# SHI-Labs/Self-Similarity-Grouping

Hardware: AMD Instinct MI355X
Metric: images/s embed + s/iter for NxN rerank+DBSCAN, N=16k, 1/2/4/8 GPU (higher is better)
Workload: dtype f32 (embed: split-half operands hi+lo on fp16 MFMA, fp32 accumulate, 6e-8 max error vs the fp32 reference features) / exact int64 via int8 MFMA digits + f64 + f16 (distance, re-rank: half semantics, bit-exact)

## Files before the change

self-similarity-grouping_amd/csrc/conv.hip:

```cpp
#include "ssg_common.h"
#include <cstdlib>
#include <type_traits>

namespace ssg {

typedef float v16f __attribute__((ext_vector_type(16)));
typedef unsigned int v4u __attribute__((ext_vector_type(4)));
typedef _Float16 v8h __attribute__((ext_vector_type(8)));

__device__ __forceinline__ unsigned pack_h2(_Float16 a, _Float16 b) {
  return (unsigned)__builtin_bit_cast(unsigned short, a) | ((unsigned)__builtin_bit_cast(unsigned short, b) << 16);
}
__device__ __forceinline__ float unpack_lo(unsigned u) { return (float)__builtin_bit_cast(_Float16, (unsigned short)(u & 0xffffu)); }
__device__ __forceinline__ float unpack_hi(unsigned u) { return (float)__builtin_bit_cast(_Float16, (unsigned short)(u >> 16)); }
__device__ __forceinline__ void split_encode4(const float4 v, uint2& hi, uint2& lo) {
  const _Float16 h0 = (_Float16)v.x, h1 = (_Float16)v.y, h2 = (_Float16)v.z, h3 = (_Float16)v.w;
  hi = make_uint2(pack_h2(h0, h1), pack_h2(h2, h3));
  lo = make_uint2(pack_h2((_Float16)(v.x - (float)h0), (_Float16)(v.y - (float)h1)), pack_h2((_Float16)(v.z - (float)h2), (_Float16)(v.w - (float)h3)));
}
__device__ __forceinline__ bool split_hi_nonfinite(const uint2 hi) {
  const unsigned a = hi.x & 0x7fff7fffu, b = hi.y & 0x7fff7fffu;
  return (a & 0xffffu) >= 0x7c00u || (a >> 16) >= 0x7c00u || (b & 0xffffu) >= 0x7c00u || (b >> 16) >= 0x7c00u;
}
__device__ __forceinline__ float4 split_decode4(const uint2 hi, const uint2 lo) {
// ... 345 lines not shown
          v.x += r4.x; v.y += r4.y; v.z += r4.z; v.w += r4.w;
        }
        if (p.relu) { v.x = v.x > 0.f ? v.x : 0.f; v.y = v.y > 0.f ? v.y : 0.f; v.z = v.z > 0.f ? v.z : 0.f; v.w = v.w > 0.f ? v.w : 0.f; }
        if (p.out_split) {
          uint2 hp, lp;
          split_encode4(v, hp, lp);
          if (p.overflow && split_hi_nonfinite(hp)) *p.overflow = 1;
          const uint2 send = odd ? hp : lp;
          const uint2 recv = make_uint2(lane_xor1(send.x), lane_xor1(send.y));
          const uint4 st = odd ? make_uint4(recv.x, recv.y, lp.x, lp.y) : make_uint4(hp.x, hp.y, recv.x, recv.y);
#ifdef SSG_IGEMM_NT_STORE
          if (m < p.M) { const v4u sv_ = {st.x, st.y, st.z, st.w}; __builtin_nontemporal_store(sv_, reinterpret_cast<v4u*>(outp + (int64_t)m * p.Cout + col)); }
#else
          if (m < p.M) *reinterpret_cast<uint4*>(outp + (int64_t)m * p.Cout + col) = st;
#endif
        } else if (m < p.M) *reinterpret_cast<float4*>(outp + (int64_t)m * p.Cout + col) = v;
      }
    }
    return;
  }
  float4 rr[MT][NT][4];
  if (resp) {
#pragma unroll
    for (int i = 0; i < MT; i++) {
      const int m = tm * BM + wm * WM + i * 32 + l32;
      const int64_t mrow = (int64_t)(m < p.M ? m : 0) * p.Cout;
#pragma unroll
      for (int j = 0; j < NT; j++)
#pragma unroll
        for (int q = 0; q < 4; q++) {
          const float* g = resp + mrow + tn * BN + wn * WN + j * 32 + 8 * q;
          if (p.res_split) {
            const uint2 hi = *reinterpret_cast<const uint2*>(g + 2 * h), lo = *reinterpret_cast<const uint2*>(g + 4 + 2 * h);
            rr[i][j][q] = make_float4(__uint_as_float(hi.x), __uint_as_float(hi.y), __uint_as_float(lo.x), __uint_as_float(lo.y));
          } else rr[i][j][q] = *reinterpret_cast<const float4*>(g + 4 * h);
        }
    }
  }
#pragma unroll
  for (int i = 0; i < MT; i++) {
    const int m = tm * BM + wm * WM + i * 32 + l32;
#pragma unroll
    for (int j = 0; j < NT; j++) {
#pragma unroll
      for (int q = 0; q < 4; q++) {
        const int col = tn * BN + wn * WN + j * 32 + 8 * q + 4 * h;
        const float4 bias = *reinterpret_cast<const float4*>(p.bias + col);
        const float4 cs = p.cscale ? *reinterpret_cast<const float4*>(p.cscale + col) : make_float4(1.f, 1.f, 1.f, 1.f);
        float4 v = make_float4(acc[i][j][4 * q] * cs.x + bias.x, acc[i][j][4 * q + 1] * cs.y + bias.y, acc[i][j][4 * q + 2] * cs.z + bias.z,
                               acc[i][j][4 * q + 3] * cs.w + bias.w);
        if (p.epi == 2) {
          v = make_float4(2.f - 2.f * acc[i][j][4 * q], 2.f - 2.f * acc[i][j][4 * q + 1], 2.f - 2.f * acc[i][j][4 * q + 2], 2.f - 2.f * acc[i][j][4 * q + 3]);
        } else if (p.epi == 1) {
          const float rt = p.rowterm[m < p.M ? m : 0];
          v = make_float4((rt + bias.x) - 2.f * acc[i][j][4 * q], (rt + bias.y) - 2.f * acc[i][j][4 * q + 1], (rt + bias.z) - 2.f * acc[i][j][4 * q + 2],
                          (rt + bias.w) - 2.f * acc[i][j][4 * q + 3]);
        }
        if (resp) {
          float4 r4 = rr[i][j][q];
          if (p.res_split) r4 = split_decode4(make_uint2(__float_as_uint(r4.x), __float_as_uint(r4.y)), make_uint2(__float_as_uint(r4.z), __float_as_uint(r4.w)));
          v.x += r4.x; v.y += r4.y; v.z += r4.z; v.w += r4.w;
        }
        if (p.relu) { v.x = v.x > 0.f ? v.x : 0.f; v.y = v.y > 0.f ? v.y : 0.f; v.z = v.z > 0.f ? v.z : 0.f; v.w = v.w > 0.f ? v.w : 0.f; }
        if (p.out_split) {
          uint2 hp, lp;
          split_encode4(v, hp, lp);
          if (p.overflow && split_hi_nonfinite(hp)) *p.overflow = 1;
          const uint2 send = h ? hp : lp;
          const uint2 recv = make_uint2((unsigned)__shfl_xor((int)send.x, 32, 64), (unsigned)__shfl_xor((int)send.y, 32, 64));
          const uint4 st = h ? make_uint4(recv.x, recv.y, lp.x, lp.y) : make_uint4(hp.x, hp.y, recv.x, recv.y);
#ifdef SSG_IGEMM_NT_STORE
          if (m < p.M) { const v4u sv_ = {st.x, st.y, st.z, st.w}; __builtin_nontemporal_store(sv_, reinterpret_cast<v4u*>(outp + (int64_t)m * p.Cout + col)); }
#else
          if (m < p.M) *reinterpret_cast<uint4*>(outp + (int64_t)m * p.Cout + col) = st;
#endif
        } else if (m < p.M) *reinterpret_cast<float4*>(outp + (int64_t)m * p.Cout + col) = v;
      }
    }
  }
}

#define SSG_LDSP(ptr_) ((__attribute__((address_space(3))) void*)(ptr_))

template <int BN, bool ONEPROD = false, int BM = 128, bool DUAL = false, int NS = 3, int WM_ = 64, bool TWOSET = false>
__global__ __launch_bounds__((BM / WM_) * (BN / 64) * 64, BM == 256 ? 1 : (BN == 256 ? 4 : 3)) void conv_dma_kernel(ConvParams p) {
  static_assert(NS == 3 || NS == 4, "three or four stages");
  static_assert(WM_ == 64 || (WM_ == 128 && BM == 256 && BN == 256 && !ONEPROD && NS == 4), "128-row wave tiles: the 256 x 256 three-product kernel");
  static_assert(!TWOSET || WM_ == 128, "second fragment set: 8-wave kernel only");
  constexpr int WM = WM_, WN = 64, MT = WM / 32, NT = 2, CBK = 16;
  constexpr int WCOLS = BN / WN, NW = (BM / WM) * WCOLS;
  constexpr int ABLK = BM / 16 / NW, WBLK = BN / 16 / NW;
  constexpr int STAGE_BYTES = (BM + BN) * 64;
  __shared__ __attribute__((aligned(1024))) unsigned char st0[STAGE_BYTES];
  __shared__ __attribute__((aligned(1024))) unsigned char st1[STAGE_BYTES];
  __shared__ __attribute__((aligned(1024))) unsigned char st2[STAGE_BYTES];
  __shared__ __attribute__((aligned(1024))) unsigned char st3[NS == 4 ? STAGE_BYTES : 1024];
  const int tiles_n = p.Cout / BN, tiles_m = (p.M + BM - 1) / BM;
  const int tile = conv_xcd_remap((int)blockIdx.x, tiles_m * tiles_n);
  const int tm = tile / tiles_n, tn = tile % tiles_n;
  const int tid = (int)threadIdx.x, lane = tid & 63, wave = __builtin_amdgcn_readfirstlane(tid >> 6);
  SSG_DMA_STAMP(0)
  const int wm = wave / WCOLS, wn = wave % WCOLS, l32 = lane & 31, h = lane >> 5;

  const int drow = lane >> 2, pc = lane & 3;
  const int lc4 = (pc ^ ((drow >> 2) & 3)) * 4;
  const int nkA = DUAL ? p.nk1 * 2 : 0x7fffffff;
  int ab0, ah0, aw0, ab1 = -1, ah1 = 0, aw1 = 0, abase0 = 0, abase1 = 0;
  unsigned a2b0 = 0x80000000u, a2b1 = 0x80000000u;
#define SSG_ROW(J)                                                                                                   \
  {                                                                                                                  \
    const int m = tm * BM + (wave * ABLK + J) * 16 + drow;                                                            \
    if (m < p.M) {                                                                                                   \
      const int b = m / (p.OH * p.OW), rem = m - b * (p.OH * p.OW);                                                  \
      const int oh = rem / p.OW, ow = rem - oh * p.OW;                                                               \
      ab##J = b; ah##J = oh * p.stride - p.pad; aw##J = ow * p.stride - p.pad;                                       \
      abase##J = (((b * p.H + ah##J) * p.W + aw##J) * p.Cin + lc4) * 4;                                               \
      if (DUAL) a2b##J = (unsigned)((((b * p.H2 + oh * p.stride2) * p.W2 + ow * p.stride2) * p.Cin2 + lc4) * 4);       \
    } else { ab##J = -1; ah##J = 0; aw##J = 0; }                                                                     \
  }
  SSG_ROW(0)
  if (ABLK == 2) SSG_ROW(1)
#undef SSG_ROW
  const __amdgpu_buffer_rsrc_t in_rsrc = __builtin_amdgcn_make_buffer_rsrc(const_cast<float*>(p.in), 0, p.in_bytes, 0x00020000);
  const __amdgpu_buffer_rsrc_t in2_rsrc = __builtin_amdgcn_make_buffer_rsrc(const_cast<float*>(p.in2 ? p.in2 : p.in), 0, p.in2 ? p.in2_bytes : 0u, 0x00020000);
#ifndef SSG_CONV_WT
#define SSG_CONV_WT 1
#endif
  const int nk = p.Kpad / CBK;
  const bool tiled = SSG_CONV_WT && !ONEPROD && p.wt != nullptr;
  const __amdgpu_buffer_rsrc_t w_rsrc = __builtin_amdgcn_make_buffer_rsrc(const_cast<float*>(tiled ? p.wt : p.w), 0, (unsigned)((int64_t)p.Cout * p.Kpad * 4), 0x00020000);
  const int wrow0 = tn * BN + wave * (16 * WBLK);
  const unsigned wo0 = tiled ? (unsigned)((((wrow0 >> 7) * nk) * 128 + (wrow0 & 127)) * 64 + lane * 16) : (unsigned)(((wrow0 + drow) * p.Kpad + lc4) * 4);
  const unsigned wo1 = wo0 + (tiled ? 1024u : (unsigned)(16 * p.Kpad * 4));
  const int wkshift = tiled ? 13 : 6;
  int dn = 0, dr = 0, ds = 0, dch = 0;
#ifndef SSG_DMA_AUX_A
#define SSG_DMA_AUX_A 0
#endif
#ifndef SSG_DMA_AUX_W
#define SSG_DMA_AUX_W 0
#endif
#define SSG_DMA_A(J, ST)                                                                                             \
  {                                                                                                                  \
    if (!DUAL || dn < nkA) {                                                                                          \
      const bool ok = ab##J >= 0 && (unsigned)(ah##J + dr) < (unsigned)p.H && (unsigned)(aw##J + ds) < (unsigned)p.W;  \
      const unsigned aoff = ok ? (unsigned)(abase##J + ddelta_) : 0x80000000u;                                        \
      __builtin_amdgcn_raw_ptr_buffer_load_lds(in_rsrc, SSG_LDSP(ST + (wave * ABLK + J) * 1024), 16, aoff, 0, 0, SSG_DMA_AUX_A);   \
    } else {                                                                                                          \
      const unsigned aoff = a2b##J + (unsigned)((dn - nkA) * CBK * 4);                                                 \
      __builtin_amdgcn_raw_ptr_buffer_load_lds(in2_rsrc, SSG_LDSP(ST + (wave * ABLK + J) * 1024), 16, aoff, 0, 0, SSG_DMA_AUX_A);  \
    }                                                                                                                 \
  }
#define SSG_DMA_NEXT(ST)                                                                                             \
  {                                                                                                                  \
    const int ddelta_ = ((dr * p.W + ds) * p.Cin + dch * 32 + (dn & 1) * 16) * 4;                                     \
    SSG_DMA_A(0, ST) if (ABLK == 2) SSG_DMA_A(1, ST)                                                                  \
    const unsigned kb_ = (unsigned)dn << wkshift;                                                                     \
    __builtin_amdgcn_raw_ptr_buffer_load_lds(w_rsrc, SSG_LDSP(ST + BM * 64 + wave * (1024 * WBLK)), 16, wo0 + kb_, 0, 0, SSG_DMA_AUX_W);   \
    if (WBLK == 2) __builtin_amdgcn_raw_ptr_buffer_load_lds(w_rsrc, SSG_LDSP(ST + BM * 64 + wave * 2048 + 1024), 16, wo1 + kb_, 0, 0, SSG_DMA_AUX_W); \
    {                                         \
      const int adv_ = dn < nk - 1 ? 1 : 0;                                                                          \
      dn += adv_;                                                                                                    \
      ds += adv_ & ~dn & 1;                                                                                          \
      const int w1_ = ds == p.KW ? 1 : 0; ds = w1_ ? 0 : ds; dr += w1_;                                               \
      const int w2_ = dr == p.KH ? 1 : 0; dr = w2_ ? 0 : dr; dch += w2_;                                              \
    }                                                                                                                \
  }

  const int g = (l32 >> 2) & 3;
  const int offh = ((2 * h) ^ g) * 16, offl = ((2 * h + 1) ^ g) * 16;
  const int arow = (wm * WM + l32) * 64, brow = BM * 64 + (wn * WN + l32) * 64;
#define SSG_MMA(ST)                                                                                                  \
  {                                                                                                                  \
    v8h ah_[MT], al_[MT], bh_[NT], bl_[NT];                                                                          \
    _Pragma("unroll") for (int i = 0; i < MT; i++) {                                                                 \
      ah_[i] = *reinterpret_cast<const v8h*>(ST + arow + i * 2048 + offh); al_[i] = *reinterpret_cast<const v8h*>(ST + arow + i * 2048 + offl); } \
    _Pragma("unroll") for (int j = 0; j < NT; j++) {                                                                 \
      bh_[j] = *reinterpret_cast<const v8h*>(ST + brow + j * 2048 + offh); bl_[j] = *reinterpret_cast<const v8h*>(ST + brow + j * 2048 + offl); } \
    if constexpr (!ONEPROD) {                                                                                        \
      _Pragma("unroll") for (int i = 0; i < MT; i++) _Pragma("unroll") for (int j = 0; j < NT; j++)                  \
        acc[i][j] = __builtin_amdgcn_mfma_f32_32x32x16_f16(bh_[j], al_[i], acc[i][j], 0, 0, 0);                      \
      _Pragma("unroll") for (int i = 0; i < MT; i++) _Pragma("unroll") for (int j = 0; j < NT; j++)                  \
        acc[i][j] = __builtin_amdgcn_mfma_f32_32x32x16_f16(bl_[j], ah_[i], acc[i][j], 0, 0, 0);                      \
    }                                                                                                                \
    _Pragma("unroll") for (int i = 0; i < MT; i++) _Pragma("unroll") for (int j = 0; j < NT; j++)                    \
      acc[i][j] = __builtin_amdgcn_mfma_f32_32x32x16_f16(bh_[j], ah_[i], acc[i][j], 0, 0, 0);                        \
  }

  v16f acc[MT][NT];
#pragma unroll
  for (int i = 0; i < MT; i++)
#pragma unroll
    for (int j = 0; j < NT; j++)
#pragma unroll
      for (int r = 0; r < 16; r++) acc[i][j][r] = 0.f;

#define SSG_PUBLISH()                                                                                              \
  { constexpr int OUTST = (ABLK + WBLK) * (NS - 2);                                                                \
    if (OUTST == 8) asm volatile("s_waitcnt vmcnt(8) lgkmcnt(0)\n\ts_barrier" ::: "memory");                                  \
    else if (OUTST == 6) asm volatile("s_waitcnt vmcnt(6) lgkmcnt(0)\n\ts_barrier" ::: "memory");                             \
    else if (OUTST == 4) asm volatile("s_waitcnt vmcnt(4) lgkmcnt(0)\n\ts_barrier" ::: "memory");                             \
    else if (OUTST == 3) asm volatile("s_waitcnt vmcnt(3) lgkmcnt(0)\n\ts_barrier" ::: "memory");                             \
    else asm volatile("s_waitcnt vmcnt(2) lgkmcnt(0)\n\ts_barrier" ::: "memory"); }
  static_assert((ABLK + WBLK) * (NS - 2) == 8 || (ABLK + WBLK) * (NS - 2) == 6 || (ABLK + WBLK) * (NS - 2) == 4 || (ABLK + WBLK) * (NS - 2) == 3 ||
                (ABLK + WBLK) * (NS - 2) == 2, "vmcnt literal for this tile shape");
#ifndef SSG_DMA_BPOS
#define SSG_DMA_BPOS 2
#endif
  constexpr int BPOS = ONEPROD ? 0 : SSG_DMA_BPOS;
  constexpr int TDMA = ABLK + WBLK;
  const int nfull = nk / NS * NS;
  if constexpr (BPOS == 0) {
  SSG_DMA_NEXT(st0)
  SSG_DMA_NEXT(st1)
  if constexpr (NS == 4) SSG_DMA_NEXT(st2)
  for (int kt = 0; kt < nfull; kt += NS) {
    if constexpr (NS == 3) {
      SSG_PUBLISH();
      SSG_DMA_NEXT(st2)
      __builtin_amdgcn_sched_barrier(0);
      SSG_MMA(st0)
      SSG_PUBLISH();
      SSG_DMA_NEXT(st0)
      __builtin_amdgcn_sched_barrier(0);
      SSG_MMA(st1)
      SSG_PUBLISH();
      SSG_DMA_NEXT(st1)
      __builtin_amdgcn_sched_barrier(0);
      SSG_MMA(st2)
    } else {
      SSG_PUBLISH();
      SSG_DMA_NEXT(st3)
      __builtin_amdgcn_sched_barrier(0);
      SSG_MMA(st0)
      SSG_PUBLISH();
      SSG_DMA_NEXT(st0)
      __builtin_amdgcn_sched_barrier(0);
      SSG_MMA(st1)
      SSG_PUBLISH();
      SSG_DMA_NEXT(st1)
      __builtin_amdgcn_sched_barrier(0);
      SSG_MMA(st2)
      SSG_PUBLISH();
      SSG_DMA_NEXT(st2)
      __builtin_amdgcn_sched_barrier(0);
      SSG_MMA(st3)
    }
  }
  if (nk - nfull >= 1) { asm volatile("s_waitcnt vmcnt(0) lgkmcnt(0)\n\ts_barrier" ::: "memory"); SSG_MMA(st0) }
  if (nk - nfull >= 2) { asm volatile("s_waitcnt vmcnt(0) lgkmcnt(0)\n\ts_barrier" ::: "memory"); SSG_MMA(st1) }
  if constexpr (NS == 4) { if (nk - nfull == 3) { asm volatile("s_waitcnt vmcnt(0) lgkmcnt(0)\n\ts_barrier" ::: "memory"); SSG_MMA(st2) } }
  } else if constexpr (TWOSET) {
    v8h fah[2][MT], fal[2][MT], fbh[2][NT], fbl[2][NT];
#define SSG_READS2(ST, S)                                                                                            \
    { _Pragma("unroll") for (int i = 0; i < MT; i++) {                                                               \
        fah[S][i] = *reinterpret_cast<const v8h*>(ST + arow + i * 2048 + offh); fal[S][i] = *reinterpret_cast<const v8h*>(ST + arow + i * 2048 + offl); } \
      _Pragma("unroll") for (int j = 0; j < NT; j++) {                                                               \
        fbh[S][j] = *reinterpret_cast<const v8h*>(ST + brow + j * 2048 + offh); fbl[S][j] = *reinterpret_cast<const v8h*>(ST + brow + j * 2048 + offl); } }
#define SSG_GA(S) { _Pragma("unroll") for (int i = 0; i < MT; i++) _Pragma("unroll") for (int j = 0; j < NT; j++)   \
      acc[i][j] = __builtin_amdgcn_mfma_f32_32x32x16_f16(fbh[S][j], fal[S][i], acc[i][j], 0, 0, 0); }
#define SSG_GB(S) { _Pragma("unroll") for (int i = 0; i < MT; i++) _Pragma("unroll") for (int j = 0; j < NT; j++)   \
      acc[i][j] = __builtin_amdgcn_mfma_f32_32x32x16_f16(fbl[S][j], fah[S][i], acc[i][j], 0, 0, 0); }
#define SSG_GC(S) { _Pragma("unroll") for (int i = 0; i < MT; i++) _Pragma("unroll") for (int j = 0; j < NT; j++)   \
      acc[i][j] = __builtin_amdgcn_mfma_f32_32x32x16_f16(fbh[S][j], fah[S][i], acc[i][j], 0, 0, 0); }
#define SSG_STEP2(ST, STN, S)                                                                                        \
    { SSG_GA(S) SSG_GB(S)                                                                                            \
      __builtin_amdgcn_sched_barrier(0);                                                                             \
      asm volatile("s_waitcnt vmcnt(%0) lgkmcnt(0)\n\ts_barrier" ::"n"(TDMA * (NS - 2)) : "memory");                  \
      SSG_DMA_NEXT(ST)                                                                                               \
      SSG_READS2(STN, 1 - (S))                                                                                       \
      __builtin_amdgcn_sched_barrier(0);                                                                             \
      SSG_GC(S) }
    SSG_DMA_NEXT(st0)
    SSG_DMA_NEXT(st1)
    SSG_DMA_NEXT(st2)
    SSG_DMA_NEXT(st3)
    asm volatile("s_waitcnt vmcnt(%0)\n\ts_barrier" ::"n"(TDMA * (NS - 1)) : "memory");
    SSG_READS2(st0, 0)
    for (int kt = 0; kt < nfull; kt += NS) {
      SSG_STEP2(st0, st1, 0)
      SSG_STEP2(st1, st2, 1)
      SSG_STEP2(st2, st3, 0)
      SSG_STEP2(st3, st0, 1)
    }
    if (nk - nfull >= 1) { SSG_GA(0) SSG_GB(0) SSG_GC(0) }
    if (nk - nfull >= 2) { asm volatile("s_waitcnt vmcnt(0) lgkmcnt(0)\n\ts_barrier" ::: "memory"); SSG_READS2(st1, 0) SSG_GA(0) SSG_GB(0) SSG_GC(0) }
    if (nk - nfull == 3) { asm volatile("s_waitcnt vmcnt(0) lgkmcnt(0)\n\ts_barrier" ::: "memory"); SSG_READS2(st2, 0) SSG_GA(0) SSG_GB(0) SSG_GC(0) }
#undef SSG_STEP2
#undef SSG_GA
#undef SSG_GB
#undef SSG_GC
#undef SSG_READS2
  } else {
    v8h fah[MT], fal[MT], fbh[NT], fbl[NT];
#define SSG_READS(ST)                                                                                                \
    { _Pragma("unroll") for (int i = 0; i < MT; i++) {                                                               \
        fah[i] = *reinterpret_cast<const v8h*>(ST + arow + i * 2048 + offh); fal[i] = *reinterpret_cast<const v8h*>(ST + arow + i * 2048 + offl); } \
      _Pragma("unroll") for (int j = 0; j < NT; j++) {                                                               \
        fbh[j] = *reinterpret_cast<const v8h*>(ST + brow + j * 2048 + offh); fbl[j] = *reinterpret_cast<const v8h*>(ST + brow + j * 2048 + offl); } }
#define SSG_G1 { _Pragma("unroll") for (int i = 0; i < MT; i++) _Pragma("unroll") for (int j = 0; j < NT; j++)      \
      acc[i][j] = __builtin_amdgcn_mfma_f32_32x32x16_f16(fbh[j], fal[i], acc[i][j], 0, 0, 0); }
#define SSG_G2 { _Pragma("unroll") for (int i = 0; i < MT; i++) _Pragma("unroll") for (int j = 0; j < NT; j++)      \
      acc[i][j] = __builtin_amdgcn_mfma_f32_32x32x16_f16(fbl[j], fah[i], acc[i][j], 0, 0, 0); }
#define SSG_G3 { _Pragma("unroll") for (int i = 0; i < MT; i++) _Pragma("unroll") for (int j = 0; j < NT; j++)      \
      acc[i][j] = __builtin_amdgcn_mfma_f32_32x32x16_f16(fbh[j], fah[i], acc[i][j], 0, 0, 0); }
#ifndef SSG_DMA_SETPRIO
#define SSG_DMA_SETPRIO 0
#endif
#if SSG_DMA_SETPRIO
#define SSG_PRIO(P_) __builtin_amdgcn_s_setprio(P_);
#else
#define SSG_PRIO(P_)
#endif
#define SSG_STEP(ST)                                                                                                 \
    { SSG_READS(ST)                                                                                                  \
      SSG_PRIO(1)                                                                                                    \
      SSG_G1                                                                                                         \
      if constexpr (BPOS == 2) SSG_G2                                                                                \
      SSG_PRIO(0)                                                                                                    \
      __builtin_amdgcn_sched_barrier(0);                                                                             \
      asm volatile("s_waitcnt vmcnt(%0) lgkmcnt(0)\n\ts_barrier" ::"n"(TDMA * (NS - 2)) : "memory");                  \
      SSG_DMA_NEXT(ST)                                                                                               \
      __builtin_amdgcn_sched_barrier(0);                                                                             \
      SSG_PRIO(1)                                                                                                    \
      if constexpr (BPOS == 1) SSG_G2                                                                                \
      SSG_G3                                                                                                         \
      SSG_PRIO(0) }
#define SSG_LAST(ST) { SSG_READS(ST) SSG_G1 SSG_G2 SSG_G3 }
    SSG_DMA_NEXT(st0)
    SSG_DMA_NEXT(st1)
    SSG_DMA_NEXT(st2)
    if constexpr (NS == 4) SSG_DMA_NEXT(st3)
    asm volatile("s_waitcnt vmcnt(%0)\n\ts_barrier" ::"n"(TDMA * (NS - 1)) : "memory");
    SSG_DMA_STAMP(1)
    for (int kt = 0; kt < nfull; kt += NS) {
      SSG_STEP(st0)
      SSG_STEP(st1)
      SSG_STEP(st2)
      if constexpr (NS == 4) SSG_STEP(st3)
    }
    if (nk - nfull >= 1) SSG_LAST(st0)
    if (nk - nfull >= 2) { asm volatile("s_waitcnt vmcnt(0) lgkmcnt(0)\n\ts_barrier" ::: "memory"); SSG_LAST(st1) }
    if constexpr (NS == 4) { if (nk - nfull == 3) { asm volatile("s_waitcnt vmcnt(0) lgkmcnt(0)\n\ts_barrier" ::: "memory"); SSG_LAST(st2) } }
#undef SSG_READS
#undef SSG_G1
#undef SSG_G2
#undef SSG_G3
#undef SSG_STEP
#undef SSG_LAST
  }
  SSG_DMA_STAMP(2)
  __syncthreads();
  SSG_DMA_STAMP(3)
#undef SSG_PUBLISH
#undef SSG_DMA_NEXT
#undef SSG_DMA_A
#undef SSG_MMA
#pragma unroll
  for (int i = 0; i < MT; i++)
#pragma unroll
    for (int j = 0; j < NT; j++)
#pragma unroll
      for (int r = 0; r < 16; r++) acc[i][j][r] *= p.acc_scale;

  if (p.epi == 3) {
#pragma unroll
    for (int i = 0; i < MT; i++) {
      const int m = tm * BM + wm * WM + i * 32 + l32;
      const float rt = p.rowterm[m < p.M ? m : 0];
#pragma unroll
      for (int j = 0; j < NT; j++) {
        float gq[4];
#pragma unroll
        for (int q = 0; q < 4; q++) {
          const float4 bias = *reinterpret_cast<const float4*>(p.bias + tn * BN + wn * WN + j * 32 + 8 * q + 4 * h);
          float mn = fminf(fminf((rt + bias.x) - 2.f * acc[i][j][4 * q], (rt + bias.y) - 2.f * acc[i][j][4 * q + 1]),
                           fminf((rt + bias.z) - 2.f * acc[i][j][4 * q + 2], (rt + bias.w) - 2.f * acc[i][j][4 * q + 3]));
          gq[q] = fminf(mn, __shfl_xor(mn, 32, 64));
        }
        if (h == 0 && m < p.M)
          *reinterpret_cast<float4*>(p.tilemin + (int64_t)m * p.tmin_ld + (tn * BN + wn * WN + j * 32) / 8) = make_float4(gq[0], gq[1], gq[2], gq[3]);
      }
    }
    return;
  }
  constexpr int EP = 36, CPR = 8, RPI = 8, ITS = 4;
  constexpr int PPS = STAGE_BYTES / (32 * EP * 4) < 6 ? STAGE_BYTES / (32 * EP * 4) : 6;
  static_assert(PPS * 32 * EP * 4 <= STAGE_BYTES && 3 * PPS >= NW, "epilogue patches fit in the stage arrays");
  float* patch = reinterpret_cast<float*>(wave < PPS ? st0 : (wave < 2 * PPS ? st1 : st2)) + (wave % PPS) * (32 * EP);
  const int chunk = lane % CPR, prow = lane / CPR, odd = lane & 1;
  const float* __restrict__ resp = p.res;
  float* __restrict__ outp = p.out;
#ifndef SSG_DMA_FAST_EPI
#define SSG_DMA_FAST_EPI 1
#endif
#ifndef SSG_DMA_RES_AUX
#define SSG_DMA_RES_AUX 2
#endif
#ifndef SSG_DMA_OUT_AUX_RES
#define SSG_DMA_OUT_AUX_RES 2
#endif
#ifndef SSG_DMA_OUT_AUX
#define SSG_DMA_OUT_AUX 0
#endif
  if (SSG_DMA_FAST_EPI && p.variant != 7 && p.out_split && p.relu && p.cscale != nullptr && (resp == nullptr || p.res_split) &&
      ((int64_t)p.M + BM) * p.Cout * 4 < (int64_t)0xffffffff) {
    constexpr int NP = MT * NT;
    unsigned ovf = 0u;
    const unsigned tbytes = (unsigned)((int64_t)p.M * p.Cout * 4), rowb = (unsigned)p.Cout * 4u;
    const __amdgpu_buffer_rsrc_t out_rsrc = __builtin_amdgcn_make_buffer_rsrc(outp, 0, tbytes, 0x00020000);
    const __amdgpu_buffer_rsrc_t res_rsrc = __builtin_amdgcn_make_buffer_rsrc(const_cast<float*>(resp ? resp : outp), 0, resp ? tbytes : 0u, 0x00020000);
    const unsigned lane_off = (unsigned)prow * rowb + (unsigned)chunk * 16u;
    const unsigned ubase = (unsigned)(tm * BM + wm * WM) * rowb + (unsigned)(tn * BN + wn * WN) * 4u;
    auto poff = [&](const int n, const int it) { return ubase + (unsigned)((n % MT) * 32 + it * RPI) * rowb + (unsigned)(n / MT) * 128u + lane_off; };
    auto run = [&](auto RES_) {
      constexpr bool RES = decltype(RES_)::value;
      v4u rr[ITS];
      v4f bias = *reinterpret_cast<const v4f*>(p.bias + tn * BN + wn * WN + chunk * 4), cs = *reinterpret_cast<const v4f*>(p.cscale + tn * BN + wn * WN + chunk * 4);
      v4f bias_n = bias, cs_n = cs;
      if constexpr (RES) {
#pragma unroll
        for (int it = 0; it < ITS; it++) rr[it] = __builtin_amdgcn_raw_buffer_load_b128(res_rsrc, poff(0, it), 0, SSG_DMA_RES_AUX);
      }
#pragma unroll
      for (int n = 0; n < NP; n++) {
        const int j = n / MT, i = n % MT;
        if (n % MT == MT - 1 && j + 1 < NT) {
          bias_n = *reinterpret_cast<const v4f*>(p.bias + tn * BN + wn * WN + (j + 1) * 32 + chunk * 4);
          cs_n = *reinterpret_cast<const v4f*>(p.cscale + tn * BN + wn * WN + (j + 1) * 32 + chunk * 4);
        }
#pragma unroll
        for (int q = 0; q < 4; q++)
          *reinterpret_cast<float4*>(patch + l32 * EP + 8 * q + 4 * h) = make_float4(acc[i][j][4 * q], acc[i][j][4 * q + 1], acc[i][j][4 * q + 2], acc[i][j][4 * q + 3]);
        __builtin_amdgcn_fence(__ATOMIC_ACQ_REL, "wavefront");
#pragma unroll
        for (int it = 0; it < ITS; it++) {
          float4 v = *reinterpret_cast<const float4*>(patch + (it * RPI + prow) * EP + chunk * 4);
          v.x = v.x * cs[0] + bias[0]; v.y = v.y * cs[1] + bias[1]; v.z = v.z * cs[2] + bias[2]; v.w = v.w * cs[3] + bias[3];
          if constexpr (RES) {
// ... 154 lines not shown
  for (int64_t x = (int64_t)blockIdx.x * blockDim.x + threadIdx.x; x < total; x += (int64_t)gridDim.x * blockDim.x) {
    const int c8 = (int)(x % C8); int64_t t = x / C8;
    const int ow = (int)(t % OW); t /= OW; const int oh = (int)(t % OH); const int b = (int)(t / OH);
    float4 m0 = make_float4(-INFINITY, -INFINITY, -INFINITY, -INFINITY), m1 = m0;
    for (int r = 0; r < 3; r++) {
      const int ih = oh * 2 - 1 + r; if (ih < 0 || ih >= H) continue;
      for (int s = 0; s < 3; s++) {
        const int iw = ow * 2 - 1 + s; if (iw < 0 || iw >= W) continue;
        float4 a, c;
        h8l8_load8(in + ((int64_t)(b * H + ih) * W + iw) * C + c8 * 8, a, c);
        m0.x = fmaxf(m0.x, a.x); m0.y = fmaxf(m0.y, a.y); m0.z = fmaxf(m0.z, a.z); m0.w = fmaxf(m0.w, a.w);
        m1.x = fmaxf(m1.x, c.x); m1.y = fmaxf(m1.y, c.y); m1.z = fmaxf(m1.z, c.z); m1.w = fmaxf(m1.w, c.w);
      }
    }
    h8l8_store8(out + x * 8, m0, m1);
  }
}

__global__ void gap_stripes_h8l8_kernel(const float* __restrict__ in, float* __restrict__ out, int B, int H, int W, int C, int S) {
  const int nsets = S > 1 ? S + 1 : 1;
  const int64_t total = (int64_t)nsets * B * C;
  const unsigned short* hp = reinterpret_cast<const unsigned short*>(in);
  for (int64_t x = (int64_t)blockIdx.x * blockDim.x + threadIdx.x; x < total; x += (int64_t)gridDim.x * blockDim.x) {
    const int c = (int)(x % C); int64_t t = x / C; const int b = (int)(t % B); const int s = (int)(t / B);
    int h0 = 0, h1 = H;
    if (s > 0) { const int hs = H / S; h0 = hs * (s - 1); h1 = hs * s; }
    float acc = 0.f;
    for (int hh = h0; hh < h1; hh++)
      for (int w = 0; w < W; w++) {
        const int64_t e = (((int64_t)(b * H + hh) * W + w) * C + (c & ~7)) * 2 + (c & 7);
        acc += (float)__builtin_bit_cast(_Float16, hp[e]) + (float)__builtin_bit_cast(_Float16, hp[e + 8]);
      }
    out[x] = acc / (float)((h1 - h0) * W);
  }
}

__global__ void h8l8_encode_kernel(const float* __restrict__ in, float* __restrict__ out, int64_t ngroups, float scale) {
  for (int64_t x = (int64_t)blockIdx.x * blockDim.x + threadIdx.x; x < ngroups; x += (int64_t)gridDim.x * blockDim.x) {
    float4 a = reinterpret_cast<const float4*>(in)[2 * x], b = reinterpret_cast<const float4*>(in)[2 * x + 1];
    a.x *= scale; a.y *= scale; a.z *= scale; a.w *= scale; b.x *= scale; b.y *= scale; b.z *= scale; b.w *= scale;
    h8l8_store8(out + x * 8, a, b);
  }
}
__global__ void h8l8_decode_kernel(const float* __restrict__ in, float* __restrict__ out, int64_t ngroups, float scale) {
  for (int64_t x = (int64_t)blockIdx.x * blockDim.x + threadIdx.x; x < ngroups; x += (int64_t)gridDim.x * blockDim.x) {
    float4 a, b;
    h8l8_load8(in + x * 8, a, b);
    a.x *= scale; a.y *= scale; a.z *= scale; a.w *= scale; b.x *= scale; b.y *= scale; b.z *= scale; b.w *= scale;
    reinterpret_cast<float4*>(out)[2 * x] = a; reinterpret_cast<float4*>(out)[2 * x + 1] = b;
  }
}

__global__ __launch_bounds__(256) void flip_sum_l2norm_kernel(const float* __restrict__ a, const float* __restrict__ b, float* __restrict__ out,
                                                              int rows, int C) {
  const int row = (int)((blockIdx.x * blockDim.x + threadIdx.x) >> 6);
  if (row >= rows) return;
  const int lane = lane_id();
  const float* pa = a + (int64_t)row * C; const float* pb = b + (int64_t)row * C;
  float ss = 0.f;
  for (int c = lane; c < C; c += 64) { const float s = pa[c] + pb[c]; ss += s * s; }
  for (int sh = 1; sh < 64; sh <<= 1) ss += __shfl_xor(ss, sh, 64);
  const float nrm = sqrtf(ss);
  for (int c = lane; c < C; c += 64) out[(int64_t)row * C + c] = (pa[c] + pb[c]) / nrm;
}

}

using namespace ssg;

template <int BM, int BN, int WM, int WN, bool CIN4, int CBK, bool SPLIT>
static int launch_conv_bk(const ConvParams& p, hipStream_t stream) {
  const size_t lds = 2 * (size_t)(BM + BN) * (CBK + 4) * sizeof(float);
  const int tiles = ((p.M + BM - 1) / BM) * (p.Cout / BN);
  static bool attr_set = false;
  if (lds > 64 * 1024 && !attr_set) {
    int rc = ssg_check_hip(hipFuncSetAttribute((const void*)conv_igemm_kernel<BM, BN, WM, WN, CIN4, CBK, SPLIT>, hipFuncAttributeMaxDynamicSharedMemorySize, (int)lds),
                           "hipFuncSetAttribute(conv)");
    if (rc) return rc;
    attr_set = true;
  }
  hipLaunchKernelGGL((conv_igemm_kernel<BM, BN, WM, WN, CIN4, CBK, SPLIT>), dim3(tiles), dim3((BM / WM) * (BN / WN) * 64), lds, stream, p);
  return ssg_check_hip(hipGetLastError(), "conv_igemm_kernel");
}
template <int BM, int BN, int WM, int WN, bool CIN4>
static int launch_conv(const ConvParams& p, hipStream_t stream, bool split = false) {
  static int bk16_max = -1;
  if (bk16_max < 0) { const char* e = getenv("SSG_CONV_BK16_MAXK"); bk16_max = e ? atoi(e) : 0x7fffffff; }
  if (split) {
    if constexpr (CIN4) return launch_conv_bk<BM, BN, WM, WN, true, 16, true>(p, stream);
    else {
      static int sbk16 = -1;
      if (sbk16 < 0) { const char* e = getenv("SSG_SPLIT_BK16"); sbk16 = e ? atoi(e) : 0; }
      if (!p.in2 && p.Kpad <= sbk16) return launch_conv_bk<BM, BN, WM, WN, false, 16, true>(p, stream);
      if constexpr (BM == 128 && BN == 128) {
        static int dma = -1;
        if (dma < 0) { const char* e = getenv("SSG_CONV_DMA"); dma = e ? atoi(e) : 3; }
        if ((dma & 2) && p.epi == 0 && !p.in2) {
          const int tiles = ((p.M + 127) / 128) * (p.Cout / 128);
          hipLaunchKernelGGL(conv_dma_kernel<128>, dim3(tiles), dim3(256), 0, stream, p);
          return ssg_check_hip(hipGetLastError(), "conv_dma_kernel<128>");
        }
      }
      return launch_conv_bk<BM, BN, WM, WN, false, 32, true>(p, stream);
    }
  }
  if (!p.in2 && p.Kpad <= bk16_max) return launch_conv_bk<BM, BN, WM, WN, CIN4, 16, false>(p, stream);
  return launch_conv_bk<BM, BN, WM, WN, CIN4, 32, false>(p, stream);
}

static bool conv_prefers_wide(const ConvParams& p, bool split) {
  static int mintiles = -1;
  if (mintiles < 0) { const char* e = getenv("SSG_SPLIT_WIDE_MINTILES"); mintiles = e ? atoi(e) : 256; }
  if (!split || mintiles <= 0 || (p.Cout % 256) || p.Kpad < 128) return false;
  return ((p.M + 127) / 128) * (p.Cout / 256) >= mintiles;
}

static int launch_conv_wide(const ConvParams& p, hipStream_t stream) {
  static int dma = -1;
  if (dma < 0) { const char* e = getenv("SSG_CONV_DMA"); dma = e ? atoi(e) : 3; }
  if ((dma & 1) && (p.epi == 0 || p.epi == 3) && (int64_t)p.Cout * p.Kpad * 4 < 0x7fffffffLL) {
    static int tall = -1;
    if (tall < 0) { const char* e = getenv("SSG_CONV_TALL_MINTILES"); tall = e ? atoi(e) : 200; }
    const int tiles_tall = ((p.M + 255) / 256) * (p.Cout / 256);
    static int tall_dual = -1;
    if (tall_dual < 0) { const char* e = getenv("SSG_CONV_TALL_DUAL"); tall_dual = e ? atoi(e) : 0; }
    if (tall > 0 && p.products == 3 && p.epi == 0 && p.in2 && tall_dual && tiles_tall >= tall) {
      hipLaunchKernelGGL((conv_dma_kernel<256, false, 256, true, 4>), dim3(tiles_tall), dim3(1024), 0, stream, p);
      return ssg_check_hip(hipGetLastError(), "conv_dma_kernel<256x256, dual>");
    }
    static int tall_res = -1;
    if (tall_res < 0) { const char* e = getenv("SSG_CONV_TALL_RES"); tall_res = e ? atoi(e) : 0; }
    if (tall > 0 && p.products == 3 && p.epi == 0 && (!p.res || tall_res) && !p.in2 && tiles_tall >= tall) {
      static int tall_ns = -1;
      if (tall_ns < 0) { const char* e = getenv("SSG_CONV_TALL_STAGES"); tall_ns = e ? atoi(e) : 4; }
      static int tall_wm = -1;
      if (tall_wm < 0) { const char* e = getenv("SSG_CONV_TALL_WM"); tall_wm = e ? atoi(e) : 64; }
      if (tall_wm == 128) hipLaunchKernelGGL((conv_dma_kernel<256, false, 256, false, 4, 128, false>), dim3(tiles_tall), dim3(512), 0, stream, p);
      else if (tall_wm == 129) hipLaunchKernelGGL((conv_dma_kernel<256, false, 256, false, 4, 128, true>), dim3(tiles_tall), dim3(512), 0, stream, p);
      else if (tall_ns == 4) hipLaunchKernelGGL((conv_dma_kernel<256, false, 256, false, 4>), dim3(tiles_tall), dim3(1024), 0, stream, p);
      else hipLaunchKernelGGL((conv_dma_kernel<256, false, 256, false>), dim3(tiles_tall), dim3(1024), 0, stream, p);
      return ssg_check_hip(hipGetLastError(), "conv_dma_kernel<256x256>");
    }
    const int tiles = ((p.M + 127) / 128) * (p.Cout / 256);
    if (p.products == 1) hipLaunchKernelGGL((conv_dma_kernel<256, true>), dim3(tiles), dim3(512), 0, stream, p);
    else if (p.in2) hipLaunchKernelGGL((conv_dma_kernel<256, false, 128, true>), dim3(tiles), dim3(512), 0, stream, p);
    else hipLaunchKernelGGL(conv_dma_kernel<256>, dim3(tiles), dim3(512), 0, stream, p);
    return ssg_check_hip(hipGetLastError(), "conv_dma_kernel");
  }
  return launch_conv_bk<128, 256, 64, 64, false, 32, true>(p, stream);
}

static bool conv_prefers_bn64(const ConvParams& p, bool split) {
  static int maxtiles = -1;
  if (maxtiles < 0) { const char* e = getenv("SSG_SPLIT_BN64_MAXTILES"); maxtiles = e ? atoi(e) : 300; }
  if (!split) return false;
  const int tiles = ((p.M + 127) / 128) * (p.Cout / 128);
  return tiles < maxtiles;
}

extern "C" int ssg_conv_weights_tile_supported(int Cout, int Kpad) { return Cout > 0 && Kpad > 0 && Cout % 128 == 0 && Kpad % 16 == 0; }

extern "C" int ssg_conv_weights_tile(const void* w, int Cout, int Kpad, void* wt, hipStream_t stream) {
  if (!ssg_conv_weights_tile_supported(Cout, Kpad)) return 0;
  if (!w || !wt || (((uintptr_t)w | (uintptr_t)wt) & 15)) { ssg_set_error("ssg_conv_weights_tile: w and wt must be given and 16-byte aligned"); return SSG_ERR_INVALID; }
  const int64_t nslots = (int64_t)Cout * Kpad / 4;
  hipLaunchKernelGGL(conv_weights_tile_kernel, dim3((unsigned)((nslots + 255) / 256)), dim3(256), 0, stream, (const uint4*)w, (uint4*)wt, Kpad / 16, nslots);
  SSG_LAUNCH_CHECK("conv_weights_tile_kernel");
  return 1;
}

static const void* conv_tiled_weights(const char* fn, const void* w, const void* wt, int flags, int Cout, int64_t Kpad, int* rc) {
  *rc = SSG_OK;
  if (!wt && (flags & 4)) wt = (const float*)w + (int64_t)Cout * Kpad;
  if (wt && (!(flags & 1) || !ssg_conv_weights_tile_supported(Cout, (int)Kpad))) {
    ssg_set_error("%s: tiled weights need split-half operands, Cout %% 128 == 0 and Kpad %% 16 == 0 (Cout=%d Kpad=%lld flags=%d)", fn, Cout, (long long)Kpad, flags);
    *rc = SSG_ERR_INVALID;
  }
  return wt;
}

extern "C" int ssg_conv2d_nhwc_xt(const void* in, const void* w, const void* wt, const float* bias, const void* res, void* out, int B, int H, int W,
                                  int Cin, int Cout, int KH, int KW, int stride, int pad, int relu, int flags, float acc_scale, const float* ch_scale,
                                  int32_t* overflow, hipStream_t stream) {
  ConvParams p;
  p.cscale = ch_scale; p.overflow = overflow;
  p.in = (const float*)in; p.w = (const float*)w; p.bias = bias; p.res = (const float*)res; p.out = (float*)out;
  p.B = B; p.H = H; p.W = W; p.Cin = Cin; p.Cout = Cout; p.KH = KH; p.KW = KW; p.stride = stride; p.pad = pad; p.relu = relu;
  p.OH = (H + 2 * pad - KH) / stride + 1; p.OW = (W + 2 * pad - KW) / stride + 1;
  const int64_t M = (int64_t)B * p.OH * p.OW;
  const bool split = (flags & 1) != 0;
  if (B <= 0 || M <= 0 || M > 0x7fffffff || (Cout % 64) || !((Cin % 32) == 0 || Cin == 4) || stride < 1) {
    ssg_set_error("ssg_conv2d_nhwc: unsupported shape B=%d H=%d W=%d Cin=%d Cout=%d k=%dx%d s=%d p=%d flags=%d", B, H, W, Cin, Cout, KH, KW, stride, pad, flags);
    return SSG_ERR_INVALID;
  }
  p.M = (int)M;
  const int64_t in_bytes = (int64_t)B * H * W * Cin * 4;
  if (in_bytes > 0x7fffffffLL) { ssg_set_error("ssg_conv2d_nhwc: input tensor of %lld bytes exceeds the 2 GiB buffer-resource range of this kernel; use a smaller batch", (long long)in_bytes); return SSG_ERR_INVALID; }
  p.in_bytes = (unsigned)in_bytes;
  p.in2 = nullptr; p.H2 = p.W2 = p.Cin2 = 0; p.stride2 = 1; p.in2_bytes = 0; p.rowterm = nullptr; p.epi = 0; p.tilemin = nullptr; p.tmin_ld = 0;
  p.out_split = (flags & 2) ? 1 : 0; p.res_split = p.out_split; p.acc_scale = acc_scale;
  static int variant = -1;
  if (variant < 0) { const char* e = getenv("SSG_CONV_VARIANT"); variant = e ? atoi(e) : 0; }
  p.variant = variant;
  const bool cin4 = (Cin == 4);
  p.Kpad = cin4 ? 32 * ((KH * KW + 7) / 8) : KH * KW * Cin;
  p.nk1 = p.Kpad / 16;
  { int rc; p.wt = (const float*)conv_tiled_weights("ssg_conv2d_nhwc_xt", w, wt, flags, Cout, p.Kpad, &rc); if (rc) return rc; }
  if (cin4) return (Cout % 128 == 0) ? launch_conv<128, 128, 64, 64, true>(p, stream, split) : launch_conv<128, 64, 64, 32, true>(p, stream, split);
  if (conv_prefers_wide(p, split)) return launch_conv_wide(p, stream);
  return (Cout % 128 == 0 && !conv_prefers_bn64(p, split)) ? launch_conv<128, 128, 64, 64, false>(p, stream, split) : launch_conv<128, 64, 64, 32, false>(p, stream, split);
}

extern "C" int ssg_conv2d_nhwc_x(const void* in, const void* w, const float* bias, const void* res, void* out, int B, int H, int W,
                                 int Cin, int Cout, int KH, int KW, int stride, int pad, int relu, int flags, float acc_scale, const float* ch_scale,
                                 int32_t* overflow, hipStream_t stream) {
  return ssg_conv2d_nhwc_xt(in, w, nullptr, bias, res, out, B, H, W, Cin, Cout, KH, KW, stride, pad, relu, flags, acc_scale, ch_scale, overflow, stream);
}

extern "C" int ssg_conv2d_nhwc_f32(const float* in, const float* w, const float* bias, const float* res, float* out, int B, int H, int W,
                                   int Cin, int Cout, int KH, int KW, int stride, int pad, int relu, hipStream_t stream) {
  return ssg_conv2d_nhwc_x(in, w, bias, res, out, B, H, W, Cin, Cout, KH, KW, stride, pad, relu, 0, 1.f, nullptr, nullptr, stream);
}

extern "C" int ssg_conv1x1_dual_nhwc_xt(const void* in, const void* in2, const void* w, const void* wt, const float* bias, void* out, int B, int H, int W,
                                        int Cin, int H2, int W2, int Cin2, int stride2, int Cout, int relu, int flags, float acc_scale, const float* ch_scale,
                                        int32_t* overflow, hipStream_t stream) {
  ConvParams p;
  p.cscale = ch_scale; p.overflow = overflow;
// ... 145 lines not shown
```

Measured before the change: 28290.

## Issue paired A-tile DMA loads covering full cache lines across two stages

Measured after the change: 28780, median of 6. +1.7%, better.

```diff
diff --git a/self-similarity-grouping_amd/csrc/conv.hip b/self-similarity-grouping_amd/csrc/conv.hip
--- a/self-similarity-grouping_amd/csrc/conv.hip
+++ b/self-similarity-grouping_amd/csrc/conv.hip
@@ -451,11 +451,16 @@
 
 #define SSG_LDSP(ptr_) ((__attribute__((address_space(3))) void*)(ptr_))
 
-template <int BN, bool ONEPROD = false, int BM = 128, bool DUAL = false, int NS = 3, int WM_ = 64, bool TWOSET = false>
+#ifndef SSG_DMA_BPOS
+#define SSG_DMA_BPOS 2
+#endif
+template <int BN, bool ONEPROD = false, int BM = 128, bool DUAL = false, int NS = 3, int WM_ = 64, bool TWOSET = false, int LINE = 0>
 __global__ __launch_bounds__((BM / WM_) * (BN / 64) * 64, BM == 256 ? 1 : (BN == 256 ? 4 : 3)) void conv_dma_kernel(ConvParams p) {
   static_assert(NS == 3 || NS == 4, "three or four stages");
   static_assert(WM_ == 64 || (WM_ == 128 && BM == 256 && BN == 256 && !ONEPROD && NS == 4), "128-row wave tiles: the 256 x 256 three-product kernel");
   static_assert(!TWOSET || WM_ == 128, "second fragment set: 8-wave kernel only");
+  static_assert(LINE == 0 || (LINE == 1 && !ONEPROD && !TWOSET), "line order: three-product kernels with one fragment set");
+  constexpr int LN = SSG_DMA_BPOS > 0 ? LINE : 0;
   constexpr int WM = WM_, WN = 64, MT = WM / 32, NT = 2, CBK = 16;
   constexpr int WCOLS = BN / WN, NW = (BM / WM) * WCOLS;
   constexpr int ABLK = BM / 16 / NW, WBLK = BN / 16 / NW;
@@ -503,6 +508,7 @@
   const unsigned wo1 = wo0 + (tiled ? 1024u : (unsigned)(16 * p.Kpad * 4));
   const int wkshift = tiled ? 13 : 6;
   int dn = 0, dr = 0, ds = 0, dch = 0;
+  [[maybe_unused]] int dnw = 0;
 #ifndef SSG_DMA_AUX_A
 #define SSG_DMA_AUX_A 0
 #endif
@@ -534,6 +540,39 @@
       const int w1_ = ds == p.KW ? 1 : 0; ds = w1_ ? 0 : ds; dr += w1_;                                               \
       const int w2_ = dr == p.KH ? 1 : 0; dr = w2_ ? 0 : dr; dch += w2_;                                              \
     }                                                                                                                \
+  }
+#define SSG_DMA_A2(J, STE, STO)                                                                                      \
+  {                                                                                                                  \
+    unsigned aoff;                                                                                                   \
+    if (!DUAL || dn < nkA) {                                                                                          \
+      const bool ok = ab##J >= 0 && (unsigned)(ah##J + dr) < (unsigned)p.H && (unsigned)(aw##J + ds) < (unsigned)p.W;  \
+      aoff = ok ? (unsigned)(abase##J + ddelta_) : 0x80000000u;                                                       \
+      __builtin_amdgcn_raw_ptr_buffer_load_lds(in_rsrc, SSG_LDSP(STE + (wave * ABLK + J) * 1024), 16, aoff, 0, 0, SSG_DMA_AUX_A);        \
+      __builtin_amdgcn_raw_ptr_buffer_load_lds(in_rsrc, SSG_LDSP(STO + (wave * ABLK + J) * 1024), 16, aoff + 64u, 0, 0, SSG_DMA_AUX_A);  \
+    } else {                                                                                                          \
+      aoff = a2b##J + (unsigned)((dn - nkA) * CBK * 4);                                                                \
+      __builtin_amdgcn_raw_ptr_buffer_load_lds(in2_rsrc, SSG_LDSP(STE + (wave * ABLK + J) * 1024), 16, aoff, 0, 0, SSG_DMA_AUX_A);       \
+      __builtin_amdgcn_raw_ptr_buffer_load_lds(in2_rsrc, SSG_LDSP(STO + (wave * ABLK + J) * 1024), 16, aoff + 64u, 0, 0, SSG_DMA_AUX_A); \
+    }                                                                                                                 \
+  }
+#define SSG_DMA_PAIR(STE, STO)                                                                                       \
+  {                                                                                                                  \
+    const int ddelta_ = ((dr * p.W + ds) * p.Cin + dch * 32) * 4;                                                     \
+    SSG_DMA_A2(0, STE, STO) if (ABLK == 2) SSG_DMA_A2(1, STE, STO)                                                    \
+    {                                                                                                                \
+      const int adv_ = dn < nk - 2 ? 1 : 0;                                                                          \
+      dn += 2 * adv_;                                                                                                \
+      ds += adv_;                                                                                                    \
+      const int w1_ = ds == p.KW ? 1 : 0; ds = w1_ ? 0 : ds; dr += w1_;                                               \
+      const int w2_ = dr == p.KH ? 1 : 0; dr = w2_ ? 0 : dr; dch += w2_;                                              \
+    }                                                                                                                \
+  }
+#define SSG_DMA_W(ST)                                                                                                \
+  {                                                                                                                  \
+    const unsigned kb_ = (unsigned)dnw << wkshift;                                                                    \
+    __builtin_amdgcn_raw_ptr_buffer_load_lds(w_rsrc, SSG_LDSP(ST + BM * 64 + wave * (1024 * WBLK)), 16, wo0 + kb_, 0, 0, SSG_DMA_AUX_W);   \
+    if (WBLK == 2) __builtin_amdgcn_raw_ptr_buffer_load_lds(w_rsrc, SSG_LDSP(ST + BM * 64 + wave * 2048 + 1024), 16, wo1 + kb_, 0, 0, SSG_DMA_AUX_W); \
+    dnw += dnw < nk - 1 ? 1 : 0;                                                                                     \
   }
 
   const int g = (l32 >> 2) & 3;
@@ -573,9 +612,6 @@
     else asm volatile("s_waitcnt vmcnt(2) lgkmcnt(0)\n\ts_barrier" ::: "memory"); }
   static_assert((ABLK + WBLK) * (NS - 2) == 8 || (ABLK + WBLK) * (NS - 2) == 6 || (ABLK + WBLK) * (NS - 2) == 4 || (ABLK + WBLK) * (NS - 2) == 3 ||
                 (ABLK + WBLK) * (NS - 2) == 2, "vmcnt literal for this tile shape");
-#ifndef SSG_DMA_BPOS
-#define SSG_DMA_BPOS 2
-#endif
   constexpr int BPOS = ONEPROD ? 0 : SSG_DMA_BPOS;
   constexpr int TDMA = ABLK + WBLK;
   const int nfull = nk / NS * NS;
@@ -696,6 +732,40 @@
       SSG_G3                                                                                                         \
       SSG_PRIO(0) }
 #define SSG_LAST(ST) { SSG_READS(ST) SSG_G1 SSG_G2 SSG_G3 }
+    if constexpr (LN == 1) {
+    constexpr int VM_PAIR = NS == 4 ? 1 + 2 * WBLK : WBLK, VM_NONE = NS == 4 ? 2 * ABLK + 2 * WBLK : 1 + WBLK;
+#define SSG_LSTEP(STP, ST, PAIR)                                                                                     \
+    { SSG_READS(ST)                                                                                                  \
+      SSG_G1                                                                                                         \
+      if constexpr (BPOS == 2) SSG_G2                                                                                \
+      __builtin_amdgcn_sched_barrier(0);                                                                             \
+      asm volatile("s_waitcnt vmcnt(%0) lgkmcnt(0)\n\ts_barrier" ::"n"((PAIR) ? VM_PAIR : VM_NONE) : "memory");       \
+      if constexpr ((PAIR) != 0) SSG_DMA_PAIR(STP, ST)                                                               \
+      SSG_DMA_W(ST)                                                                                                  \
+      __builtin_amdgcn_sched_barrier(0);                                                                             \
+      if constexpr (BPOS == 1) SSG_G2                                                                                \
+      SSG_G3 }
+    if constexpr (NS == 4) {
+      SSG_DMA_W(st0)
+      SSG_DMA_PAIR(st0, st1) SSG_DMA_W(st1)
+      SSG_DMA_W(st2)
+      SSG_DMA_PAIR(st2, st3) SSG_DMA_W(st3)
+      asm volatile("s_waitcnt vmcnt(%0)\n\ts_barrier" ::"n"(1 + 2 * ABLK + 3 * WBLK) : "memory");
+      int kt = 0;
+      for (; kt + 4 <= nk; kt += 4) { SSG_LSTEP(st3, st0, 0) SSG_LSTEP(st0, st1, 1) SSG_LSTEP(st1, st2, 0) SSG_LSTEP(st2, st3, 1) }
+      if (nk - kt >= 2) { SSG_LSTEP(st3, st0, 0) SSG_LSTEP(st0, st1, 1) }
+    } else {
+      SSG_DMA_W(st0)
+      SSG_DMA_PAIR(st0, st1) SSG_DMA_W(st1)
+      SSG_DMA_W(st2)
+      asm volatile("s_waitcnt vmcnt(%0)\n\ts_barrier" ::"n"(1 + 2 * WBLK) : "memory");
+      int kt = 0;
+      for (; kt + 6 <= nk; kt += 6) { SSG_LSTEP(st2, st0, 1) SSG_LSTEP(st0, st1, 0) SSG_LSTEP(st1, st2, 1) SSG_LSTEP(st2, st0, 0) SSG_LSTEP(st0, st1, 1) SSG_LSTEP(st1, st2, 0) }
+      if (nk - kt >= 2) { SSG_LSTEP(st2, st0, 1) SSG_LSTEP(st0, st1, 0) }
+      if (nk - kt >= 4) { SSG_LSTEP(st1, st2, 1) SSG_LSTEP(st2, st0, 0) }
+    }
+#undef SSG_LSTEP
+    } else {
     SSG_DMA_NEXT(st0)
     SSG_DMA_NEXT(st1)
     SSG_DMA_NEXT(st2)
@@ -711,6 +781,7 @@
     if (nk - nfull >= 1) SSG_LAST(st0)
     if (nk - nfull >= 2) { asm volatile("s_waitcnt vmcnt(0) lgkmcnt(0)\n\ts_barrier" ::: "memory"); SSG_LAST(st1) }
     if constexpr (NS == 4) { if (nk - nfull == 3) { asm volatile("s_waitcnt vmcnt(0) lgkmcnt(0)\n\ts_barrier" ::: "memory"); SSG_LAST(st2) } }
+    }
 #undef SSG_READS
 #undef SSG_G1
 #undef SSG_G2
@@ -724,6 +795,9 @@
 #undef SSG_PUBLISH
 #undef SSG_DMA_NEXT
 #undef SSG_DMA_A
+#undef SSG_DMA_PAIR
+#undef SSG_DMA_A2
+#undef SSG_DMA_W
 #undef SSG_MMA
 #pragma unroll
   for (int i = 0; i < MT; i++)
@@ -1044,6 +1118,16 @@
   hipLaunchKernelGGL((conv_igemm_kernel<BM, BN, WM, WN, CIN4, CBK, SPLIT>), dim3(tiles), dim3((BM / WM) * (BN / WN) * 64), lds, stream, p);
   return ssg_check_hip(hipGetLastError(), "conv_igemm_kernel");
 }
+enum ConvDmaInst { DMA_128 = 0, DMA_WIDE, DMA_WIDE_DUAL, DMA_TALL, DMA_TALL_DUAL };
+static int conv_line_order(const ConvParams& p, ConvDmaInst inst) {
+  static int knob = -2;
+  if (knob == -2) { const char* e = getenv("SSG_CONV_LINE"); knob = e ? (atoi(e) == 1 ? 1 : 0) : -1; }
+  if (p.products != 3 || p.epi != 0 || ((p.Kpad / 16) & 1) || (p.Cin % 32) || (p.in2 && (p.Cin2 % 32))) return 0;
+  if (knob >= 0) return knob;
+  static const int dflt[5] = {1, 1, 1, 1, 0};
+  return dflt[inst];
+}
+
 template <int BM, int BN, int WM, int WN, bool CIN4>
 static int launch_conv(const ConvParams& p, hipStream_t stream, bool split = false) {
   static int bk16_max = -1;
@@ -1059,7 +1143,8 @@
         if (dma < 0) { const char* e = getenv("SSG_CONV_DMA"); dma = e ? atoi(e) : 3; }
         if ((dma & 2) && p.epi == 0 && !p.in2) {
           const int tiles = ((p.M + 127) / 128) * (p.Cout / 128);
-          hipLaunchKernelGGL(conv_dma_kernel<128>, dim3(tiles), dim3(256), 0, stream, p);
+          if (conv_line_order(p, DMA_128)) hipLaunchKernelGGL((conv_dma_kernel<128, false, 128, false, 3, 64, false, 1>), dim3(tiles), dim3(256), 0, stream, p);
+          else hipLaunchKernelGGL(conv_dma_kernel<128>, dim3(tiles), dim3(256), 0, stream, p);
           return ssg_check_hip(hipGetLastError(), "conv_dma_kernel<128>");
         }
       }
@@ -1087,7 +1172,8 @@
     static int tall_dual = -1;
     if (tall_dual < 0) { const char* e = getenv("SSG_CONV_TALL_DUAL"); tall_dual = e ? atoi(e) : 0; }
     if (tall > 0 && p.products == 3 && p.epi == 0 && p.in2 && tall_dual && tiles_tall >= tall) {
-      hipLaunchKernelGGL((conv_dma_kernel<256, false, 256, true, 4>), dim3(tiles_tall), dim3(1024), 0, stream, p);
+      if (conv_line_order(p, DMA_TALL_DUAL)) hipLaunchKernelGGL((conv_dma_kernel<256, false, 256, true, 4, 64, false, 1>), dim3(tiles_tall), dim3(1024), 0, stream, p);
+      else hipLaunchKernelGGL((conv_dma_kernel<256, false, 256, true, 4>), dim3(tiles_tall), dim3(1024), 0, stream, p);
       return ssg_check_hip(hipGetLastError(), "conv_dma_kernel<256x256, dual>");
     }
     static int tall_res = -1;
@@ -1099,13 +1185,16 @@
       if (tall_wm < 0) { const char* e = getenv("SSG_CONV_TALL_WM"); tall_wm = e ? atoi(e) : 64; }
       if (tall_wm == 128) hipLaunchKernelGGL((conv_dma_kernel<256, false, 256, false, 4, 128, false>), dim3(tiles_tall), dim3(512), 0, stream, p);
       else if (tall_wm == 129) hipLaunchKernelGGL((conv_dma_kernel<256, false, 256, false, 4, 128, true>), dim3(tiles_tall), dim3(512), 0, stream, p);
+      else if (tall_ns == 4 && conv_line_order(p, DMA_TALL)) hipLaunchKernelGGL((conv_dma_kernel<256, false, 256, false, 4, 64, false, 1>), dim3(tiles_tall), dim3(1024), 0, stream, p);
       else if (tall_ns == 4) hipLaunchKernelGGL((conv_dma_kernel<256, false, 256, false, 4>), dim3(tiles_tall), dim3(1024), 0, stream, p);
       else hipLaunchKernelGGL((conv_dma_kernel<256, false, 256, false>), dim3(tiles_tall), dim3(1024), 0, stream, p);
       return ssg_check_hip(hipGetLastError(), "conv_dma_kernel<256x256>");
     }
     const int tiles = ((p.M + 127) / 128) * (p.Cout / 256);
     if (p.products == 1) hipLaunchKernelGGL((conv_dma_kernel<256, true>), dim3(tiles), dim3(512), 0, stream, p);
+    else if (p.in2 && conv_line_order(p, DMA_WIDE_DUAL)) hipLaunchKernelGGL((conv_dma_kernel<256, false, 128, true, 3, 64, false, 1>), dim3(tiles), dim3(512), 0, stream, p);
     else if (p.in2) hipLaunchKernelGGL((conv_dma_kernel<256, false, 128, true>), dim3(tiles), dim3(512), 0, stream, p);
+    else if (conv_line_order(p, DMA_WIDE)) hipLaunchKernelGGL((conv_dma_kernel<256, false, 128, false, 3, 64, false, 1>), dim3(tiles), dim3(512), 0, stream, p);
     else hipLaunchKernelGGL(conv_dma_kernel<256>, dim3(tiles), dim3(512), 0, stream, p);
     return ssg_check_hip(hipGetLastError(), "conv_dma_kernel");
   }
```
